# peterWon/GLoc3D

Hardware: AMD Instinct MI355X
Metric: localization queries/sec (kNN+top-20 reg), KITTI-00-sized DB (higher is better)
Workload: dtype f32

## Files before the change

### gloc3d_amd/capi.py

```python
import ctypes as C
import os

import numpy as np

HERE = os.path.dirname(os.path.abspath(__file__))
LIB_PATH = os.environ.get("GLOC3D_LIB_PATH") or os.path.join(HERE, "lib", "libgloc3d.so")

GLOC_OK = 0
ERR_NAMES = {1: "GLOC_ERR_INVALID", 2: "GLOC_ERR_HIP", 3: "GLOC_ERR_NOMEM", 4: "GLOC_ERR_NODEVICE",
             5: "GLOC_ERR_STATE"}
ALGO_AUTO, ALGO_EXACT, ALGO_MFMA, ALGO_MFMA_FP32 = 0, 1, 2, 3
KNN_OPT_ALGO, KNN_OPT_CANDIDATES, KNN_OPT_PROFILE = 1, 2, 3
REG_OPT_PROFILE, REG_OPT_NN_MODE, REG_OPT_NN_SRC_PER_LANE, REG_OPT_NN_JOB_GROUP, REG_OPT_TEMP_TARGET_INDEX = 1, 2, 3, 4, 5
REG_OPT_NN_SPLIT_HELPERS, REG_OPT_NN_SPLIT_THRESH, REG_OPT_NN_SUB_JOBS, REG_OPT_NN_HEAVY_THRESH, REG_OPT_SUB_BATCHES = 6, 7, 8, 9, 10
REG_OPT_NN_CHAIN = 11
REG_OPT_PAIRGRAPH_BUDGET = 12
REG_NN_CULLED, REG_NN_EXHAUSTIVE = 0, 1
NO_SCAN = 0xFFFFFFFF
SIZE_MAX = C.c_size_t(-1).value


class GlocError(RuntimeError):
    def __init__(self, code, msg):
        super().__init__(f"{ERR_NAMES.get(code, code)}: {msg}")
        self.code = code


class RaycastParams(C.Structure):
    _fields_ = [("n_beams", C.c_uint32), ("n_az", C.c_uint32), ("max_range", C.c_double), ("noise_sigma", C.c_double),
                ("fov_lo_deg", C.c_double), ("fov_hi_deg", C.c_double)]


class KnnStats(C.Structure):
    _fields_ = [("searches_exact", C.c_uint64), ("searches_mfma", C.c_uint64),
                ("queries_total", C.c_uint64), ("queries_fallback", C.c_uint64),
                ("last_n_tile", C.c_uint32), ("last_k_split", C.c_uint32),
                ("last_candidates", C.c_uint32)]


class RegParams(C.Structure):
    _fields_ = [("ransac_iters", C.c_uint32), ("inlier_thresh", C.c_float),
                ("min_inlier_ratio", C.c_float), ("icp_iters", C.c_uint32),
                ("max_corr_dist", C.c_float), ("seed", C.c_uint64),
                ("ransac_confidence", C.c_float), ("max_rmse", C.c_float), ("max_final_step", C.c_float)]


class NdtParams(C.Structure):
    _fields_ = [("source_leaf", C.c_float), ("resolution", C.c_float), ("step_size", C.c_float), ("trans_eps", C.c_float),
                ("max_iters", C.c_uint32), ("outlier_ratio", C.c_float), ("min_points_per_cell", C.c_uint32),
                ("min_covar_eigvalue_mult", C.c_float)]


class P2lParams(C.Structure):
    _fields_ = [("max_iters", C.c_uint32), ("max_corr_dist", C.c_float), ("trans_eps", C.c_float), ("rot_eps", C.c_float),
                ("normal_k", C.c_uint32), ("reserved_", C.c_uint32)]


class GicpParams(C.Structure):
    _fields_ = [("max_iters", C.c_uint32), ("max_corr_dist", C.c_float), ("trans_eps", C.c_float), ("rot_eps", C.c_float),
                ("normal_k", C.c_uint32), ("plane_eps", C.c_float)]


class VgicpParams(C.Structure):
    _fields_ = [("max_iters", C.c_uint32), ("max_corr_dist", C.c_float), ("trans_eps", C.c_float), ("rot_eps", C.c_float),
                ("normal_k", C.c_uint32), ("plane_eps", C.c_float), ("resolution", C.c_float), ("neighbors", C.c_uint32),
                ("min_points", C.c_uint32), ("reserved_", C.c_uint32)]


class FpfhParams(C.Structure):
# ... 993 lines not shown
    def ransac_hypotheses(self, src, tgt, corr, seed, cand, n_hyp, inlier_thresh):
        s = np.ascontiguousarray(src, np.float32).reshape(-1, 3)
        t = np.ascontiguousarray(tgt, np.float32).reshape(-1, 3)
        c = np.ascontiguousarray(corr, np.uint32)
        Rt = np.empty((n_hyp, 12), np.float32)
        valid = np.empty(n_hyp, np.uint32)
        inl = np.empty(n_hyp, np.uint32)
        check(lib().gloc_reg_ransac_hypotheses(self._h, _np_ptr(s), _np_ptr(t), _np_ptr(c),
                                               s.shape[0], seed, cand, n_hyp, _np_ptr(Rt),
                                               _np_ptr(valid), _np_ptr(inl), inlier_thresh))
        return Rt, valid, inl

    def final_steps(self, n_jobs):
        out = np.empty(n_jobs, np.float32)
        check(lib().gloc_reg_final_steps(self._h, _np_ptr(out), n_jobs))
        return out

    def nn_stats(self):
        c, n = C.c_uint64(), C.c_uint64()
        check(lib().gloc_reg_nn_stats(self._h, C.byref(c), C.byref(n)))
        return c.value, n.value

    def debug_chain(self):
        f = lib().gloc_reg_debug_chain
        f.restype = C.c_int
        f.argtypes = [C.c_void_p, C.POINTER(C.c_uint64), C.POINTER(C.c_uint64)]
        n, t = C.c_uint64(), C.c_uint64()
        check(f(self._h, C.byref(n), C.byref(t)))
        return n.value, t.value

    def debug_needed_iters(self, inl, n, conf, max_iters):
        f = lib().gloc_reg_debug_needed_iters
        f.restype = C.c_int
        f.argtypes = [C.c_void_p, C.c_void_p, C.c_void_p, C.c_uint32, C.c_float, C.c_uint32, C.c_void_p]
        a, b = np.ascontiguousarray(inl, np.uint32), np.ascontiguousarray(n, np.uint32)
        out = np.empty(a.shape[0], np.uint32)
        check(f(self._h, _np_ptr(a), _np_ptr(b), a.shape[0], conf, max_iters, _np_ptr(out)))
        return out

    def debug_chain_stall(self, on):
        f = lib().gloc_reg_debug_chain_stall
        f.restype = C.c_int
        f.argtypes = [C.c_void_p, C.c_int]
        check(f(self._h, 1 if on else 0))

    def debug_corr(self, job, n_src):
        f = lib().gloc_reg_debug_corr
        f.restype = C.c_int
        f.argtypes = [C.c_void_p, C.c_uint32, C.c_uint32, C.c_void_p, C.c_void_p]
        idx, d2 = np.empty(n_src, np.uint32), np.empty(n_src, np.float32)
        check(f(self._h, job, n_src, _np_ptr(idx), _np_ptr(d2)))
        return idx, d2


def reg_select_first_ok(ok):
    a = np.ascontiguousarray(ok, np.int32)
    return lib().gloc_reg_select_first_ok(_np_ptr(a), a.shape[0])


class NetVladFC(_Handle):

    _C = "vlad"
    set_stream, set_profile, profile = _set_stream, _set_profile, _profile

    def __init__(self, conv_w, centroids, fc_w, conv_b=None, normalize_input=True, device=0):
        cw = np.ascontiguousarray(conv_w, np.float32)
        ce = np.ascontiguousarray(centroids, np.float32)
        fw = np.ascontiguousarray(fc_w, np.float32)
        cb = None if conv_b is None else np.ascontiguousarray(conv_b, np.float32)
        self.K, self.C = cw.shape
        self.out_dim = fw.shape[1]
        assert ce.shape == (self.K, self.C) and fw.shape[0] == self.K * self.C
        self._h = C.c_void_p()
        check(lib().gloc_vlad_create(device, self.C, self.K, self.out_dim, _np_ptr(cw),
                                     None if cb is None else _np_ptr(cb), _np_ptr(ce), _np_ptr(fw),
                                     1 if normalize_input else 0, C.byref(self._h)))

    def set_gating(self, gating_w=None, scale=None, shift=None):
        if gating_w is None:
            check(lib().gloc_vlad_set_gating(self._h, None, None, None))
            return
        gw = np.ascontiguousarray(gating_w, np.float32)
        sc = np.ascontiguousarray(scale, np.float32)
        sh = np.ascontiguousarray(shift, np.float32)
        assert gw.shape == (self.out_dim, self.out_dim) and sc.shape == (self.out_dim,) == sh.shape
        check(lib().gloc_vlad_set_gating(self._h, _np_ptr(gw), _np_ptr(sc), _np_ptr(sh)))

    def forward(self, feat):
        x = np.ascontiguousarray(feat, np.float32)
        n = x.shape[0]
        x = x.reshape(n, self.C, -1)
        out = np.empty((n, self.out_dim), np.float32)
        check(lib().gloc_vlad_forward(self._h, _np_ptr(x), n, x.shape[2], _np_ptr(out)))
        return out

    def forward_device(self, feat_ptr, n, hw, out_ptr):
        check(lib().gloc_vlad_forward_device(self._h, C.c_void_p(feat_ptr), n, hw, C.c_void_p(out_ptr)))


def default_bev_params(**over):
    p = BevParams()
    check(lib().gloc_bev_default_params(C.byref(p)))
    for k, v in over.items():
        if k == "pad_bgr":
            for i in range(3):
                p.pad_bgr[i] = v[i]
# ... 458 lines not shown
```

### gloc3d_amd/csrc/reg.hip

```cpp
#include <algorithm>
#include <cmath>
#include <vector>

#include "common.hpp"

#include "fpfh.hpp"
#include "ndt.hpp"
#include "nn_compact.hpp"
#include "gicp.hpp"
#include "p2l.hpp"
#include "pairgraph.hpp"
#include "reg_kernels.hpp"
#include "scan_store.hpp"
#include "vgicp.hpp"

using namespace gloc;
using namespace gloc::reg;

struct gloc_reg : Handle {
  hipEvent_t done_ev = nullptr;
  gloc_scan_store* store = nullptr;
  gloc_scan_store* own_store = nullptr;
  DevBuf jobs, states;
  DevBuf corr, d2, pairs;
  DevBuf Rt, valid, inliers;
  DevBuf alive;
  DevBuf partials;
  DevBuf export_idx, export_d2;
  DevBuf counters;
  void* pin = nullptr;
  size_t pin_cap = 0;
  CandState* h_states = nullptr;
  Job* h_jobs = nullptr;
  struct Pending {
    bool active = false;
    std::vector<size_t> slot;
    std::vector<size_t> n_src;
    std::vector<float> def_T;
    size_t total = 0;
    float max_rmse = 0.f, max_final_step = 0.f;
    bool icp = false;
    gloc_scan_store* store = nullptr;
    std::vector<uint32_t> pinned;
  } pending;
  std::vector<float> last_final_step;
  int nn_mode = 0;
  int nn_src_per_lane = 2;
  int nn_job_group = 24;
  bool nn_job_group_set = false;
  int nn_sub_jobs = 0;
  bool temp_target_index = false;
  int nn_split_helpers = -1;
  uint32_t nn_split_thresh = 60000;
  bool nn_split_thresh_set = false;
  DevBuf split_zero, split_ff;
  NnSplit split{};
  int nn_heavy_thresh = 32;
  DevBuf heavy_buf;
  size_t heavy_cap = 0;
  NnHeavy heavy{};
  std::atomic<uint64_t> nn_launches{0};
  int nn_chain = 1;
  bool chain_broken = false;
  bool chain_stall = false;
  DevBuf chain_buf;
  uint32_t* h_chain_err = nullptr;
  bool chain_in_batch = false;
  std::vector<unsigned char> retry_jobs;
  std::vector<float> retry_T;
  gloc_reg_params retry_prm{};
  std::atomic<uint64_t> chain_launches{0}, chain_timeouts{0};
  size_t last_ld = 0;
  uint32_t last_jobs = 0;
  gloc::ndt::Ws* ndt = nullptr;
  gloc::p2l::Ws* p2l = nullptr;
  gloc::vgicp::Ws* vgicp = nullptr;
  gloc::fpfh::Ws* fpfh = nullptr;
  gloc::pairgraph::Ws* pgraph = nullptr;
  size_t pgraph_budget = 0;
  ~gloc_reg() {
    if (pending.active && pending.store) store_pin(pending.store, pending.pinned.data(), pending.pinned.size(), -1);
    if (store) store->attached--;
    if (own_store) (void)gloc_scan_store_destroy(own_store);
    gloc::ndt::ws_free(ndt);
    gloc::p2l::ws_free(p2l);
    gloc::vgicp::ws_free(vgicp);
// ... 213 lines not shown

bool batch_chains(const gloc_reg* h, const BatchDims& bd, uint32_t hx, uint32_t warm_passes) {
  if (!h->nn_chain || h->chain_broken || h->nn_mode == 1 || h->nn_src_per_lane != 2 || h->prof.enabled || NN_WPB != 1) return false;
  if (hx == 0 || warm_passes < 2) return false;
  uint32_t jg, subs;
  launch_order(h, bd.n_jobs, jg, subs);
  if (bd.n_jobs >= 48 || (jg & 7u) || jg % subs) return false;
  if ((bd.n_part & 31u) || (hx & 31u)) return false;
  const uint32_t n_wg = ((bd.max_groups + hx + NN_WPB - 1) / NN_WPB + subs - 1) / subs;
  const uint32_t groups = (bd.n_jobs * subs + jg - 1) / jg;
  const uint64_t grp_size = ((uint64_t)jg * n_wg + (jg / subs) * NN_CHAIN_ROLES + 7) & ~7ull;
  return grp_size * groups * warm_passes < (1ull << 31);
}

int launch_nn_chain(gloc_reg* h, const BatchDims& bd, const WsView& v, uint32_t n_pass, float gate2) {
  uint32_t jg, subs;
  launch_order(h, v.n_jobs, jg, subs);
  const uint32_t n_wg = ((bd.max_groups + v.split.hx + NN_WPB - 1) / NN_WPB + subs - 1) / subs;
  const uint32_t groups = (v.n_jobs * subs + jg - 1) / jg;
  NnChain ch{};
  ch.n_pass = n_pass;
  ch.expected = subs * n_wg * NN_WPB + (h->chain_stall ? 1u : 0u);
  ch.jobs_per_grp = jg / subs;
  ch.grp_size = (jg * n_wg + ch.jobs_per_grp * NN_CHAIN_ROLES + 7u) & ~7u;
  ch.pass_size = ch.grp_size * groups;
  const size_t cells = (size_t)n_pass * v.n_jobs, line = NN_CHAIN_PAD * 4;
  const size_t head = (4 * cells + 1) * line;
  const size_t t_bytes = cells * NN_CHAIN_T_STRIDE * 4;
  const size_t plan_bytes = (size_t)(n_pass - 1) * v.n_jobs * bd.n_part * 4, help_bytes = (size_t)(n_pass - 1) * v.n_jobs * v.split.hx * 4;
  const size_t sub_bytes = sizeof(double) * ACC_NV * NN_CHAIN_RED * v.n_jobs;
  GLOC_TRY(h->chain_buf.ensure(head + t_bytes + plan_bytes + help_bytes + sub_bytes + 256, v.s));
  GLOC_HIP(hipMemsetAsync(h->chain_buf.p, 0, head, v.s));
  char* base = h->chain_buf.as<char>();
  ch.ready = reinterpret_cast<uint32_t*>(base);
  ch.done = reinterpret_cast<uint32_t*>(base + cells * line);
  ch.go = reinterpret_cast<uint32_t*>(base + 2 * cells * line);
  ch.sdone = reinterpret_cast<uint32_t*>(base + 3 * cells * line);
  ch.err = reinterpret_cast<uint32_t*>(base + 4 * cells * line);
  ch.Tp = reinterpret_cast<float*>(base + head);
  ch.planp = reinterpret_cast<uint32_t*>(base + head + t_bytes);
  ch.helperp = reinterpret_cast<uint32_t*>(base + head + t_bytes + plan_bytes);
  ch.sub = reinterpret_cast<double*>(base + head + t_bytes + plan_bytes + help_bytes);
  h->nn_launches += n_pass;
  h->chain_launches++;
  h->chain_in_batch = true;
  const NnArgs a{v, bd, jg, n_wg, subs, gate2, nullptr};
  launch_compact<nn_chain_kernel<2>>(a, dim3(ch.pass_size * n_pass), v.corr, false, NnHeavy{}, ch);
  GLOC_HIP(hipGetLastError());
  GLOC_HIP(hipMemcpyAsync(h->h_chain_err, ch.err, 4, hipMemcpyDeviceToHost, v.s));
  return GLOC_OK;
}

int ensure_pinned(gloc_reg* h, uint32_t n_jobs) {
  const size_t need = (sizeof(CandState) + sizeof(Job)) * (size_t)n_jobs + 64;
  if (need > h->pin_cap) {
    if (h->pin) (void)hipHostFree(h->pin);
    h->pin = nullptr;
    h->pin_cap = 0;
    const size_t cap = need + need / 2 + 4096;
    GLOC_HIP(hipHostMalloc(&h->pin, cap, hipHostMallocDefault));
    h->pin_cap = cap;
  }
  h->h_states = reinterpret_cast<CandState*>(h->pin);
  h->h_jobs = reinterpret_cast<Job*>(h->h_states + n_jobs);
  h->h_chain_err = reinterpret_cast<uint32_t*>(h->h_jobs + n_jobs);
  return GLOC_OK;
}

struct BatchSpec {
  uint32_t n_jobs, max_src;
  uint32_t max_groups;
  bool search;
  bool pairs;
  size_t hyp;
  bool alive;
  uint32_t split_hx;
  uint32_t warm_passes;
  static BatchSpec searching(uint32_t n_jobs, size_t max_src, uint32_t max_groups) {
    return BatchSpec{n_jobs, (uint32_t)max_src, max_groups, true, false, 0, false, 0u, 0u};
  }
  static BatchSpec on_pairs(uint32_t n_jobs, size_t max_src, size_t hyp, bool alive) {
    return BatchSpec{n_jobs, (uint32_t)max_src, 0u, false, true, hyp, alive, 0u, 0u};
  }
};

struct Batch {
  BatchDims bd;
  uint32_t nblocks;
  bool chained;
  WsView v;
};

template <class Fill>
int open_batch(gloc_reg* h, const BatchSpec& sp, Batch* out, Fill&& fill) {
  const uint32_t n_jobs = sp.n_jobs;
  const int cs = h->nn_src_per_lane;
  hipStream_t s = h->stream;
  Batch& b = *out;
  b = Batch{};
  BatchDims& bd = b.bd;
  bd = BatchDims{n_jobs, sp.max_src, sp.max_groups, 0, 0};
  b.nblocks = (bd.max_src + ACC_PER_BLOCK - 1) / ACC_PER_BLOCK;
  bd.n_part = (std::max<uint32_t>(std::max(bd.max_groups, b.nblocks), 1) + 31u) & ~31u;
  bd.ld = ((size_t)bd.max_src + 127) & ~(size_t)127;
  h->last_jobs = 0;
  GLOC_TRY(ensure_pinned(h, n_jobs));
  h->chain_in_batch = false;
  *h->h_chain_err = 0u;
  fill(h->h_jobs, h->h_states);
  WsView& v = b.v;
  v.s = s;
  v.n_jobs = n_jobs;
  GLOC_TRY(h->jobs.ensure(sizeof(Job) * n_jobs, s));
  GLOC_TRY(h->states.ensure(sizeof(CandState) * n_jobs, s));
  GLOC_TRY(h->partials.ensure(sizeof(double) * ACC_NV * (size_t)bd.n_part * n_jobs, s));
  v.jobs = h->jobs.as<Job>();
  v.states = h->states.as<CandState>();
  v.partials = h->partials.as<double>();
// ... 112 lines not shown
                         (const uint32_t*)nullptr, 0u, chunk_len);
    }
    if (ph + 1 < n_ph)
      hipLaunchKernelGGL(ransac_scan_kernel<false>, dim3(n_jobs), dim3(64), 0, s, v.inliers,
                         v.valid, v.Rt, H, h0, h1, v.jobs, r.confidence,
                         r.min_inlier_ratio, v.states);
    else
      hipLaunchKernelGGL(ransac_scan_kernel<true>, dim3(n_jobs), dim3(64), 0, s, v.inliers,
                         v.valid, v.Rt, H, h0, h1, v.jobs, r.confidence,
                         r.min_inlier_ratio, v.states);
    GLOC_HIP(hipGetLastError());
  }
  return enqueue_refit(h, bd, v, thr2, nblocks);
}

int enqueue_pipeline(gloc_reg* h, const BatchDims& bd, const gloc_reg_params* prm, const WsView& v, bool can, bool any_tgt,
                     uint32_t nblocks, bool chained) {
  const uint32_t n_jobs = v.n_jobs;
  hipStream_t s = v.s;
  const bool culled = h->nn_mode != 1;
  const float gate2 = prm->max_corr_dist > 0.f ? prm->max_corr_dist * prm->max_corr_dist : 0.f;
  bool have_corr = false;

  if (can && any_tgt && prm->ransac_iters > 0) {
    GLOC_TRY(launch_nn(h, bd, v, false, true, 0.f));
    have_corr = true;
    GLOC_TRY(enqueue_ransac(h, bd, RansacRule{prm->ransac_iters, prm->inlier_thresh, prm->min_inlier_ratio, prm->ransac_confidence, prm->seed},
                            v, nblocks));
  }
  for (uint32_t it = 0; it < prm->icp_iters && can && any_tgt; ++it) {
    if (chained && have_corr) {
      GLOC_TRY(launch_nn_chain(h, bd, v, prm->icp_iters - it, gate2));
      break;
    }
    GLOC_TRY(launch_nn(h, bd, v, have_corr, false, gate2));
    have_corr = true;
    if (!culled) {
      ProfScope ps(h->prof, "accum", s);
      hipLaunchKernelGGL(accum_kernel<0>, dim3(nblocks, n_jobs), dim3(ACC_THREADS), 0, s, v.jobs,
                         v.states, v.corr, v.d2,
                         (const f32x4*)nullptr, bd.ld, gate2, v.partials, bd.n_part);
      GLOC_HIP(hipGetLastError());
    }
    {
      ProfScope ps(h->prof, "solve", s);
      hipLaunchKernelGGL(solve_kernel<0>, dim3(v.split.hx ? 2 * n_jobs : n_jobs), dim3(SOLVE_THREADS), 0, s, v.partials,
                         bd.n_part, culled, v.jobs, v.states, v.split, n_jobs);
      GLOC_HIP(hipGetLastError());
    }
  }
  return GLOC_OK;
}

int enqueue_jobs(gloc_reg* h, const std::vector<JobHost>& jh, const gloc_reg_params* prm) {
  const uint32_t n_jobs = (uint32_t)jh.size();
  if (n_jobs == 0) return GLOC_OK;
  const int cs = h->nn_src_per_lane;
  uint32_t max_src = 0;
  bool can = false, any_tgt = false;
  for (const JobHost& j : jh) {
    max_src = std::max<uint32_t>(max_src, (uint32_t)j.src.n);
    can |= j.src.n >= 3;
    any_tgt |= j.tgt.n >= 1;
  }
  const bool ransac = can && any_tgt && prm->ransac_iters > 0;
  const bool adaptive = prm->ransac_confidence > 0.f && prm->ransac_confidence < 1.f;
  const uint32_t warm_passes = !(can && any_tgt) ? 0u : (ransac ? prm->icp_iters : std::max<uint32_t>(prm->icp_iters, 1u) - 1u);
  BatchSpec spec = BatchSpec::searching(n_jobs, max_src, src_groups(max_src, cs));
  spec.pairs = ransac;
  spec.hyp = prm->ransac_iters;
  spec.alive = !adaptive;
  spec.split_hx = split_helpers(h, n_jobs);
  spec.warm_passes = warm_passes;
  Batch b;
  GLOC_TRY(open_batch(h, spec, &b, [&](Job* jd, CandState* st) {
    for (uint32_t c = 0; c < n_jobs; ++c) {
      const DevScan &s = jh[c].src, &t = jh[c].tgt;
      jd[c] = Job{s.idx.pts, s.order, s.idx.inv, t.xyz, t.idx, (uint32_t)s.n, src_groups(s.n, cs), jh[c].stream_id, 0u};
      init_state(st[c], jh[c].init_T, prm->ransac_iters);
      if (s.n < 3) st[c].frozen = 1;
    }
  }));
  hipStream_t s = h->stream;
  GLOC_TRY(enqueue_pipeline(h, b.bd, prm, b.v, can, any_tgt, b.nblocks, b.chained));
  GLOC_HIP(hipMemcpyAsync(h->h_states, h->states.p, sizeof(CandState) * n_jobs, hipMemcpyDeviceToHost, s));
  GLOC_HIP(hipEventRecord(h->done_ev, s));
  if (h->chain_in_batch) {
    h->retry_jobs.resize(sizeof(JobHost) * n_jobs);
    memcpy(h->retry_jobs.data(), jh.data(), sizeof(JobHost) * n_jobs);
    h->retry_T.assign((size_t)16 * n_jobs, 0.f);
    for (uint32_t c = 0; c < n_jobs; ++c)
      if (jh[c].init_T) memcpy(&h->retry_T[(size_t)16 * c], jh[c].init_T, sizeof(float) * 16);
    h->retry_prm = *prm;
  }
  return GLOC_OK;
}

int collect_jobs(gloc_reg* h, uint32_t n_jobs, const size_t* n_src_of, float max_rmse, float max_final_step, float* out_T,
                 float* out_rmse, uint32_t* out_inliers, int* out_ok) {
  h->last_final_step.assign(n_jobs, 0.f);
  if (n_jobs == 0) return GLOC_OK;
  GLOC_HIP(hipEventSynchronize(h->done_ev));
  if (h->chain_in_batch && *h->h_chain_err) {
    const bool first = !h->chain_broken;
    h->chain_broken = true;
    h->chain_timeouts++;
    if (first)
      fprintf(stderr, "[gloc3d] the chained ICP passes of a batch of %u jobs timed out on the device (a wait for a job's solve ran out): "
                      "the batch is run again launch by launch, and this handle launches pass by pass from now on\n", n_jobs);
    GLOC_REQUIRE(h->retry_jobs.size() == sizeof(JobHost) * n_jobs, GLOC_ERR_HIP,
                 "the chained ICP passes of a batch of %u jobs timed out on the device and the batch cannot be run again", n_jobs);
    std::vector<JobHost> jh(n_jobs);
    memcpy(jh.data(), h->retry_jobs.data(), sizeof(JobHost) * n_jobs);
    for (uint32_t c = 0; c < n_jobs; ++c)
      if (jh[c].init_T) jh[c].init_T = &h->retry_T[(size_t)16 * c];
    const gloc_reg_params prm = h->retry_prm;
    if (const int rc = enqueue_jobs(h, jh, &prm)) {
      (void)hipStreamSynchronize(h->stream);
      return rc;
    }
    GLOC_HIP(hipEventSynchronize(h->done_ev));
  }
  for (uint32_t c = 0; c < n_jobs; ++c) {
    const CandState& st = h->h_states[c];
    const size_t n_src = n_src_of[c];
    pose_to_T16(st, out_T + 16 * (size_t)c);
    const float rmse = n_src ? (float)std::sqrt(st.sum_d2 / (double)n_src) : 0.f;
    if (out_rmse) out_rmse[c] = rmse;
    if (out_inliers) out_inliers[c] = st.best_inl;
    h->last_final_step[c] = st.last_step;
    if (out_ok)
      out_ok[c] = st.ok && !(max_rmse > 0.f && !(rmse <= max_rmse)) && !(max_final_step > 0.f && !(st.last_step <= max_final_step));
  }
  return GLOC_OK;
}

int run_jobs(gloc_reg* h, const std::vector<JobHost>& jh, const gloc_reg_params* prm, float* out_T, float* out_rmse,
             uint32_t* out_inliers, int* out_ok) {
  GLOC_TRY(enqueue_jobs(h, jh, prm));
  std::vector<size_t> n_src(jh.size());
  for (size_t c = 0; c < jh.size(); ++c) n_src[c] = jh[c].src.n;
  return collect_jobs(h, (uint32_t)jh.size(), n_src.data(), prm->max_rmse, prm->icp_iters ? prm->max_final_step : 0.f, out_T,
                      out_rmse, out_inliers, out_ok);
}

// ... 418 lines not shown
  }
  if (option == GLOC_REG_OPT_NN_MODE) {
    GLOC_REQUIRE(value == GLOC_REG_NN_CULLED || value == GLOC_REG_NN_EXHAUSTIVE, GLOC_ERR_INVALID,
                 "bad nn mode %lld", (long long)value);
    h->nn_mode = (int)value;
    return GLOC_OK;
  }
  if (option == GLOC_REG_OPT_NN_JOB_GROUP) {
    GLOC_REQUIRE(value >= 1 && value <= 65536, GLOC_ERR_INVALID, "must be in [1, 65536]");
    h->nn_job_group = (int)value;
    h->nn_job_group_set = true;
    return GLOC_OK;
  }
  if (option == GLOC_REG_OPT_TEMP_TARGET_INDEX) {
    h->temp_target_index = value != 0;
    return GLOC_OK;
  }
  if (option == GLOC_REG_OPT_NN_SUB_JOBS) {
    GLOC_REQUIRE(value >= 0 && value <= 64, GLOC_ERR_INVALID, "must be in [0, 64]");
    h->nn_sub_jobs = (int)value;
    return GLOC_OK;
  }
  if (option == GLOC_REG_OPT_NN_SPLIT_HELPERS) {
    GLOC_REQUIRE(value >= -1 && value <= 4096, GLOC_ERR_INVALID, "must be in [-1, 4096]");
    h->nn_split_helpers = (int)value;
    return GLOC_OK;
  }
  if (option == GLOC_REG_OPT_SUB_BATCHES) {
    GLOC_REQUIRE(value >= -1 && value <= 8, GLOC_ERR_INVALID, "must be in [-1, 8]");
    return GLOC_OK;
  }
  if (option == GLOC_REG_OPT_NN_CHAIN) {
    GLOC_REQUIRE(value == 0 || value == 1, GLOC_ERR_INVALID, "must be 0 or 1");
    h->nn_chain = (int)value;
    if (value) h->chain_broken = false;
    return GLOC_OK;
  }
  if (option == GLOC_REG_OPT_NN_HEAVY_THRESH) {
    GLOC_REQUIRE(value >= 0 && value <= 65535, GLOC_ERR_INVALID, "must be in [0, 65535]");
    h->nn_heavy_thresh = (int)value;
    return GLOC_OK;
  }
  if (option == GLOC_REG_OPT_NN_SPLIT_THRESH) {
    GLOC_REQUIRE(value >= 0 && value <= 0x3FFFFFFF, GLOC_ERR_INVALID, "must be in [0, 2^30)");
    h->nn_split_thresh = (uint32_t)value;
    h->nn_split_thresh_set = true;
    return GLOC_OK;
  }
  if (option == GLOC_REG_OPT_NN_SRC_PER_LANE) {
    GLOC_REQUIRE(value == 1 || value == 2 || value == 4, GLOC_ERR_INVALID, "must be 1, 2 or 4");
    h->nn_src_per_lane = (int)value;
    return GLOC_OK;
  }
  if (option == GLOC_REG_OPT_PAIRGRAPH_BUDGET) {
    GLOC_REQUIRE(value >= 0 && (uint64_t)value <= gloc::pairgraph::BUDGET_BYTES, GLOC_ERR_INVALID, "must be in [0, 2^30]");
    h->pgraph_budget = (size_t)value;
    return GLOC_OK;
  }
  set_err("unknown option %d", option);
  return GLOC_ERR_INVALID;
}

int gloc_reg_scan_upload(gloc_reg* h, const float* pts, size_t n, size_t stride_floats,
                         uint32_t* scan_id) {
  GLOC_REQUIRE(h, GLOC_ERR_INVALID, "null handle");
  GLOC_HIP(hipSetDevice(h->device));
  GLOC_TRY(ensure_store(h));
  return gloc_scan_store_add(h->store, pts, n, stride_floats, scan_id);
}

int gloc_reg_scan_build_target_index(gloc_reg* h, uint32_t scan_id) {
  GLOC_REQUIRE(h, GLOC_ERR_INVALID, "null handle");
  GLOC_REQUIRE(h->store, GLOC_ERR_INVALID, "unknown scan id %u", scan_id);
  GLOC_HIP(hipSetDevice(h->device));
  GLOC_HIP(hipStreamSynchronize(h->stream));
  return gloc_scan_store_build_target_index(h->store, scan_id);
}

int gloc_reg_scan_release(gloc_reg* h, uint32_t scan_id) {
  GLOC_REQUIRE(h, GLOC_ERR_INVALID, "null handle");
  GLOC_REQUIRE(h->store, GLOC_ERR_INVALID, "unknown scan id %u", scan_id);
  GLOC_HIP(hipSetDevice(h->device));
  GLOC_HIP(hipStreamSynchronize(h->stream));
  return gloc_scan_store_release(h->store, scan_id);
}

int gloc_reg_scan_count(const gloc_reg* h, size_t* n_scans) {
  GLOC_REQUIRE(h && n_scans, GLOC_ERR_INVALID, "null argument");
  *n_scans = 0;
  if (!h->store) return GLOC_OK;
  return gloc_scan_store_count(h->store, n_scans);
}

int gloc_reg_batch(gloc_reg* h, const float* q_xyz, size_t nq_pts, const float* const* cand_xyz,
                   const size_t* cand_npts, size_t n_cand, const uint32_t* cand_stream_ids,
                   const float* init_T, const gloc_reg_params* params, float* out_T,
                   float* out_rmse, uint32_t* out_inliers, int* out_ok) {
  GLOC_REQUIRE(h && out_T && (q_xyz || nq_pts == 0), GLOC_ERR_INVALID, "null argument");
  GLOC_REQUIRE(n_cand >= 1 && n_cand <= 4096 && cand_xyz && cand_npts, GLOC_ERR_INVALID,
               "n_cand = %zu outside [1,4096] or null candidate arrays", n_cand);
  GLOC_REQUIRE(nq_pts < (1ull << 31), GLOC_ERR_INVALID, "query scan too large");
  GLOC_NOT_PENDING(h);
  GLOC_TRY(check_params(params));
  GLOC_HIP(hipSetDevice(h->device));
  for (size_t c = 0; c < n_cand; ++c) {
    GLOC_REQUIRE(cand_xyz[c] || cand_npts[c] == 0, GLOC_ERR_INVALID, "candidate %zu is null", c);
// ... 280 lines not shown
  GLOC_HIP(hipMemcpyAsync(v.pairs, hp.data(), sizeof(float) * hp.size(), hipMemcpyHostToDevice, s));
  GLOC_HIP(hipMemsetAsync(v.inliers, 0, sizeof(uint32_t) * (size_t)n_hyp, s));
  hipLaunchKernelGGL(ransac_hyp_kernel, dim3((n_hyp + 127) / 128, 1), dim3(128), 0, s, v.pairs, ld, v.jobs, seed, n_hyp, 0u, n_hyp,
                     (const CandState*)nullptr, v.Rt, v.valid);
  GLOC_HIP(hipGetLastError());
  dim3 grid((n_hyp + 255) / 256, (unsigned)((n + SC_CHUNK - 1) / SC_CHUNK), 1);
  hipLaunchKernelGGL(ransac_score_kernel, grid, dim3(256), 0, s, v.pairs, ld, v.jobs, n_hyp, 0u, 256u , v.Rt,
                     v.valid, inlier_thresh * inlier_thresh, (const CandState*)nullptr, v.inliers, (const uint32_t*)nullptr,
                     (const uint32_t*)nullptr, 0u, (uint32_t)SC_CHUNK);
  GLOC_HIP(hipGetLastError());
  GLOC_HIP(hipMemcpyAsync(out_Rt, v.Rt, sizeof(float) * 12 * (size_t)n_hyp, hipMemcpyDeviceToHost, s));
  GLOC_HIP(hipMemcpyAsync(out_valid, v.valid, sizeof(uint32_t) * (size_t)n_hyp, hipMemcpyDeviceToHost, s));
  GLOC_HIP(hipMemcpyAsync(out_inliers, v.inliers, sizeof(uint32_t) * (size_t)n_hyp, hipMemcpyDeviceToHost, s));
  GLOC_HIP(hipStreamSynchronize(s));
  return GLOC_OK;
}

int gloc_reg_nn_stats(gloc_reg* h, uint64_t* pairs_evaluated, uint64_t* launches) {
  GLOC_REQUIRE(h, GLOC_ERR_INVALID, "null handle");
  GLOC_HIP(hipSetDevice(h->device));
  unsigned long long c = 0;
  if (h->counters.p) {
    std::vector<unsigned long long> part(NN_STAT_SLOTS);
    GLOC_HIP(hipMemcpyAsync(part.data(), h->counters.p, 8 * NN_STAT_SLOTS, hipMemcpyDeviceToHost, h->stream));
    GLOC_HIP(hipStreamSynchronize(h->stream));
    for (unsigned long long v : part) c += v;
  }
  if (pairs_evaluated) *pairs_evaluated = c;
  if (launches) *launches = h->nn_launches;
  return GLOC_OK;
}

int gloc_reg_debug_corr(gloc_reg* h, uint32_t job, uint32_t n_src, uint32_t* out_idx, float* out_d2) {
  GLOC_REQUIRE(h && out_idx && out_d2, GLOC_ERR_INVALID, "null argument");
  GLOC_HIP(hipSetDevice(h->device));
  hipStream_t s = h->stream;
  const size_t ld = h->last_ld;
  GLOC_NOT_PENDING(h);
  GLOC_REQUIRE(job < h->last_jobs && n_src <= ld, GLOC_ERR_INVALID, "no such job in the last batch");
  GLOC_TRY(h->export_idx.ensure(sizeof(uint32_t) * ld * h->last_jobs, s));
  GLOC_TRY(h->export_d2.ensure(sizeof(float) * ld * h->last_jobs, s));
  hipLaunchKernelGGL(export_corr_kernel, dim3((unsigned)((ld + 255) / 256), h->last_jobs), dim3(256), 0, s,
                     h->jobs.as<Job>(), h->corr.as<uint32_t>(), h->d2.as<float>(), ld,
                     h->export_idx.as<uint32_t>(), h->export_d2.as<float>());
  GLOC_HIP(hipGetLastError());
  GLOC_HIP(hipMemcpyAsync(out_idx, h->export_idx.as<uint32_t>() + (size_t)job * ld, sizeof(uint32_t) * n_src,
                          hipMemcpyDeviceToHost, s));
  GLOC_HIP(hipMemcpyAsync(out_d2, h->export_d2.as<float>() + (size_t)job * ld, sizeof(float) * n_src,
                          hipMemcpyDeviceToHost, s));
  GLOC_HIP(hipStreamSynchronize(s));
  return GLOC_OK;
}

int gloc_reg_debug_chain(gloc_reg* h, uint64_t* launches, uint64_t* timeouts) {
  GLOC_REQUIRE(h, GLOC_ERR_INVALID, "null handle");
  if (launches) *launches = h->chain_launches;
  if (timeouts) *timeouts = h->chain_timeouts;
  return GLOC_OK;
}

int gloc_reg_debug_needed_iters(gloc_reg* h, const uint32_t* inl, const uint32_t* n, uint32_t count, float conf, uint32_t max_iters,
                                uint32_t* out) {
  GLOC_REQUIRE(h && inl && n && out, GLOC_ERR_INVALID, "null argument");
  GLOC_HIP(hipSetDevice(h->device));
  GLOC_NOT_PENDING(h);
  hipStream_t s = h->stream;
  GLOC_TRY(h->export_idx.ensure(sizeof(uint32_t) * 3 * (size_t)count, s));
  uint32_t* d = h->export_idx.as<uint32_t>();
  GLOC_HIP(hipMemcpyAsync(d, inl, 4 * (size_t)count, hipMemcpyHostToDevice, s));
  GLOC_HIP(hipMemcpyAsync(d + count, n, 4 * (size_t)count, hipMemcpyHostToDevice, s));
  hipLaunchKernelGGL(needed_iters_kernel, dim3((count + 255) / 256), dim3(256), 0, s, d, d + count, conf, max_iters, d + 2 * (size_t)count, count);
  GLOC_HIP(hipGetLastError());
  GLOC_HIP(hipMemcpyAsync(out, d + 2 * (size_t)count, 4 * (size_t)count, hipMemcpyDeviceToHost, s));
  GLOC_HIP(hipStreamSynchronize(s));
  return GLOC_OK;
}

int gloc_reg_debug_chain_stall(gloc_reg* h, int on) {
  GLOC_REQUIRE(h, GLOC_ERR_INVALID, "null handle");
  h->chain_stall = on != 0;
  return GLOC_OK;
}

int gloc_reg_ndt_batch_ids(gloc_reg* h, uint32_t src_scan_id, const uint32_t* tgt_scan_ids, size_t n, const float* init_T,
                           const gloc_ndt_params* prm, float* out_T, double* out_prob, uint32_t* out_iters,
                           int* out_converged) {
  GLOC_REQUIRE(h && out_T && tgt_scan_ids, GLOC_ERR_INVALID, "null argument");
  GLOC_NOT_PENDING(h);
  GLOC_HIP(hipSetDevice(h->device));
  return gloc::ndt::run(ndt_ctx(h), src_scan_id, tgt_scan_ids, n, init_T, nullptr, prm, out_T, out_prob, out_iters, out_converged,
                        nullptr);
}

int gloc_reg_ndt_derivatives(gloc_reg* h, uint32_t src_scan_id, uint32_t tgt_scan_id, const double p6[6],
                             const gloc_ndt_params* prm, double* out_score, double* out_grad6, double* out_hess36) {
  GLOC_REQUIRE(h && p6 && out_score && out_grad6 && out_hess36, GLOC_ERR_INVALID, "null argument");
  GLOC_NOT_PENDING(h);
  GLOC_HIP(hipSetDevice(h->device));
  double s[43];
  GLOC_TRY(gloc::ndt::run(ndt_ctx(h), src_scan_id, &tgt_scan_id, 1, nullptr, p6, prm, nullptr, nullptr, nullptr, nullptr, s));
  *out_score = s[0];
  for (int i = 0; i < 6; ++i) out_grad6[i] = s[1 + i];
  for (int i = 0; i < 36; ++i) out_hess36[i] = s[7 + i];
  return GLOC_OK;
}

// ... 161 lines not shown
```

### include/gloc3d.h

```cpp
#ifndef GLOC3D_H
#define GLOC3D_H

#include <stddef.h>
#include <stdint.h>

#ifdef __cplusplus
extern "C" {
#endif

#define GLOC3D_ABI_VERSION 6

enum {
  GLOC_OK = 0,
  GLOC_ERR_INVALID = 1,
  GLOC_ERR_HIP = 2,
  GLOC_ERR_NOMEM = 3,
  GLOC_ERR_NODEVICE = 4,
  GLOC_ERR_STATE = 5
};

const char* gloc_last_error(void);
int gloc_abi_version(void);
int gloc_device_count(void);

// ... 51 lines not shown
int gloc_knn_search_sharded(gloc_knn* h, gloc_comm* comm, const float* d_queries, size_t nq, size_t k,
                            uint64_t index_stride, uint64_t index_offset, uint64_t* d_out_idx,
                            float* d_out_d2);

int gloc_knn_search_sharded_host(gloc_knn* h, gloc_comm* comm, const float* queries, size_t nq, size_t k,
                                 uint64_t index_stride, uint64_t index_offset, uint64_t* out_idx,
                                 float* out_d2);
int gloc_comm_all_gather_host(gloc_comm* c, const void* send, void* recv, size_t bytes_per_rank);

typedef struct gloc_knn_stats {
  uint64_t searches_exact, searches_mfma, queries_total, queries_fallback;
  uint32_t last_n_tile, last_k_split, last_candidates;
} gloc_knn_stats;
int gloc_knn_get_stats(const gloc_knn* h, gloc_knn_stats* out);

int gloc_knn_profile(gloc_knn* h, const char* kernel, double* total_ms, uint64_t* launches);
int gloc_knn_profile_reset(gloc_knn* h);

typedef struct gloc_reg gloc_reg;

typedef struct gloc_reg_params {
  uint32_t ransac_iters;
  float inlier_thresh;
  float min_inlier_ratio;
  uint32_t icp_iters;
  float max_corr_dist;
  uint64_t seed;
  float ransac_confidence;
  float max_rmse;
  float max_final_step;
} gloc_reg_params;

#define GLOC_REG_FINAL_STEP_SUGGESTED 0.03f

void gloc_reg_default_params(gloc_reg_params* p);

int gloc_reg_create(int device, gloc_reg** out);
int gloc_reg_destroy(gloc_reg* h);
int gloc_reg_set_stream(gloc_reg* h, void* hip_stream);
int gloc_reg_synchronize(gloc_reg* h);
int gloc_reg_set_option(gloc_reg* h, int option, int64_t value);
enum {
  GLOC_REG_OPT_PROFILE = 1,
  GLOC_REG_OPT_NN_MODE = 2,
  GLOC_REG_OPT_NN_SRC_PER_LANE = 3,
  GLOC_REG_OPT_NN_JOB_GROUP = 4,
  GLOC_REG_OPT_TEMP_TARGET_INDEX = 5,
  GLOC_REG_OPT_NN_SPLIT_HELPERS = 6,
  GLOC_REG_OPT_NN_SPLIT_THRESH = 7,
  GLOC_REG_OPT_NN_SUB_JOBS = 8,
  GLOC_REG_OPT_NN_HEAVY_THRESH = 9,
  GLOC_REG_OPT_SUB_BATCHES = 10,
  GLOC_REG_OPT_NN_CHAIN = 11,
  GLOC_REG_OPT_PAIRGRAPH_BUDGET = 12
};
enum {
  GLOC_REG_NN_CULLED = 0,
  GLOC_REG_NN_EXHAUSTIVE = 1
};

typedef struct gloc_scan_store gloc_scan_store;
int gloc_scan_store_create(int device, gloc_scan_store** out);
int gloc_scan_store_destroy(gloc_scan_store* st);
int gloc_scan_store_add(gloc_scan_store* st, const float* pts, size_t n, size_t stride_floats,
                        uint32_t* scan_id);
int gloc_scan_store_add_device(gloc_scan_store* st, const float* d_pts, size_t n,
                               size_t stride_floats, uint32_t* scan_id);
int gloc_scan_store_add_batch(gloc_scan_store* st, const float* const* pts, const size_t* n, size_t count,
                              size_t stride_floats, uint32_t* scan_ids);
int gloc_scan_store_build_target_index(gloc_scan_store* st, uint32_t scan_id);
int gloc_scan_store_build_target_index_batch(gloc_scan_store* st, const uint32_t* scan_ids, size_t count);
int gloc_scan_store_release(gloc_scan_store* st, uint32_t scan_id);
int gloc_scan_store_clear(gloc_scan_store* st);
int gloc_scan_store_count(gloc_scan_store* st, size_t* n_scans);
int gloc_scan_store_bytes(gloc_scan_store* st, size_t* live_bytes, size_t* cached_bytes);
int gloc_scan_store_points(gloc_scan_store* st, uint32_t scan_id, size_t* n_points);
int gloc_scan_store_download(gloc_scan_store* st, uint32_t scan_id, float* out_xyz,
                             size_t capacity_points);
int gloc_scan_store_build_normals(gloc_scan_store* st, uint32_t scan_id, uint32_t k );
int gloc_scan_store_normals(gloc_scan_store* st, uint32_t scan_id, float* out_nxyz, size_t capacity_points);

int gloc_reg_attach_store(gloc_reg* h, gloc_scan_store* store);

int gloc_reg_scan_upload(gloc_reg* h, const float* pts, size_t n, size_t stride_floats,
                         uint32_t* scan_id);
int gloc_reg_scan_build_target_index(gloc_reg* h, uint32_t scan_id);
int gloc_reg_scan_release(gloc_reg* h, uint32_t scan_id);
int gloc_reg_scan_count(const gloc_reg* h, size_t* n_scans);
int gloc_reg_scan_clear(gloc_reg* h);

int gloc_reg_batch(gloc_reg* h, const float* q_xyz, size_t nq_pts, const float* const* cand_xyz,
                   const size_t* cand_npts, size_t n_cand, const uint32_t* cand_stream_ids,
                   const float* init_T, const gloc_reg_params* params, float* out_T,
                   float* out_rmse, uint32_t* out_inliers, int* out_ok);

int gloc_reg_batch_ids(gloc_reg* h, uint32_t q_scan_id, const uint32_t* cand_scan_ids,
                       size_t n_cand, const uint32_t* cand_stream_ids, const float* init_T,
                       const gloc_reg_params* params, float* out_T, float* out_rmse,
                       uint32_t* out_inliers, int* out_ok);

int gloc_reg_batch_multi(gloc_reg* h, size_t n_queries, const uint32_t* q_scan_ids,
                         const uint32_t* cand_scan_ids, size_t n_cand,
                         const uint32_t* cand_stream_ids, const float* init_T,
                         const gloc_reg_params* params, float* out_T, float* out_rmse,
                         uint32_t* out_inliers, int* out_ok);

int gloc_reg_batch_multi_begin(gloc_reg* h, size_t n_queries, const uint32_t* q_scan_ids,
// ... 396 lines not shown
```

Measured before the change: 593.7.

## Regroup source points spatially per batch and sort groups by extent for NN

Result: faster. 601.5 (median of 6 runs) (+1.3%).

```diff
diff --git a/gloc3d_amd/capi.py b/gloc3d_amd/capi.py
--- a/gloc3d_amd/capi.py
+++ b/gloc3d_amd/capi.py
@@ -15,6 +15,7 @@
 REG_OPT_NN_SPLIT_HELPERS, REG_OPT_NN_SPLIT_THRESH, REG_OPT_NN_SUB_JOBS, REG_OPT_NN_HEAVY_THRESH, REG_OPT_SUB_BATCHES = 6, 7, 8, 9, 10
 REG_OPT_NN_CHAIN = 11
 REG_OPT_PAIRGRAPH_BUDGET = 12
+REG_OPT_SRC_GROUPING = 13
 REG_NN_CULLED, REG_NN_EXHAUSTIVE = 0, 1
 NO_SCAN = 0xFFFFFFFF
 SIZE_MAX = C.c_size_t(-1).value
@@ -1114,6 +1115,20 @@
         check(f(self._h, job, n_src, _np_ptr(idx), _np_ptr(d2)))
         return idx, d2
 
+    def debug_src_view(self, scan_id, n, src_per_lane=2, batch=None):
+        f = lib().gloc_reg_debug_src_view
+        f.restype = C.c_int
+        f.argtypes = [C.c_void_p, C.c_void_p, C.c_size_t, C.c_size_t, C.c_void_p, C.c_void_p, C.POINTER(C.c_int)]
+        ids = np.ascontiguousarray([scan_id] if batch is None else batch, np.uint32)
+        which = int(np.nonzero(ids == scan_id)[0][0])
+        ng = (n + 64 * src_per_lane - 1) // (64 * src_per_lane)
+        perm, order = np.empty(max(n, 1), np.uint32), np.empty(max(ng, 1), np.uint32)
+        has = C.c_int()
+        check(f(self._h, _np_ptr(ids), ids.shape[0], which, _np_ptr(perm), _np_ptr(order), C.byref(has)))
+        if not has.value:
+            return None
+        return dict(perm=perm[:n], order=order[:ng])
+
 
 def reg_select_first_ok(ok):
     a = np.ascontiguousarray(ok, np.int32)
diff --git a/gloc3d_amd/csrc/reg.hip b/gloc3d_amd/csrc/reg.hip
--- a/gloc3d_amd/csrc/reg.hip
+++ b/gloc3d_amd/csrc/reg.hip
@@ -1,5 +1,6 @@
 #include <algorithm>
 #include <cmath>
+#include <map>
 #include <vector>
 
 #include "common.hpp"
@@ -12,6 +13,8 @@
 #include "pairgraph.hpp"
 #include "reg_kernels.hpp"
 #include "scan_store.hpp"
+#include "seg_sort.hpp"
+#include "src_view.hpp"
 #include "vgicp.hpp"
 
 using namespace gloc;
@@ -32,6 +35,9 @@
   size_t pin_cap = 0;
   CandState* h_states = nullptr;
   Job* h_jobs = nullptr;
+  SrcView* h_views = nullptr;
+  int src_grouping = 1;
+  DevBuf view_pts, view_idx, view_desc;
   struct Pending {
     bool active = false;
     std::vector<size_t> slot;
@@ -351,7 +357,7 @@
 }
 
 int ensure_pinned(gloc_reg* h, uint32_t n_jobs) {
-  const size_t need = (sizeof(CandState) + sizeof(Job)) * (size_t)n_jobs + 64;
+  const size_t need = (sizeof(CandState) + sizeof(Job) + sizeof(SrcView) + sizeof(segsort::Seg)) * (size_t)n_jobs + 64;
   if (need > h->pin_cap) {
     if (h->pin) (void)hipHostFree(h->pin);
     h->pin = nullptr;
@@ -363,6 +369,7 @@
   h->h_states = reinterpret_cast<CandState*>(h->pin);
   h->h_jobs = reinterpret_cast<Job*>(h->h_states + n_jobs);
   h->h_chain_err = reinterpret_cast<uint32_t*>(h->h_jobs + n_jobs);
+  h->h_views = reinterpret_cast<SrcView*>(reinterpret_cast<char*>(h->h_jobs + n_jobs) + 64);
   return GLOC_OK;
 }
 
@@ -581,10 +588,78 @@
   return GLOC_OK;
 }
 
-int enqueue_jobs(gloc_reg* h, const std::vector<JobHost>& jh, const gloc_reg_params* prm) {
+int build_src_views(gloc_reg* h, std::vector<JobHost>& jh, int cs) {
+  if (!h->src_grouping || h->nn_mode == 1) return GLOC_OK;
+  hipStream_t s = h->stream;
   const uint32_t n_jobs = (uint32_t)jh.size();
+  GLOC_TRY(ensure_pinned(h, n_jobs));
+  std::vector<segsort::Seg> segs;
+  std::vector<uint32_t> view_of(n_jobs, 0xFFFFFFFFu);
+  std::map<const void*, uint32_t> seen;
+  std::vector<size_t> pts_off;
+  size_t n_pts = 0;
+  uint32_t n_views = 0, max_blocks = 0, n_grp = 0;
+  for (uint32_t c = 0; c < n_jobs; ++c) {
+    const DevScan& sc = jh[c].src;
+    const uint32_t ng = src_groups(sc.n, cs);
+    if (sc.kd || sc.n == 0 || !sc.order || ng > SV_MAX_GROUPS) continue;
+    auto it = seen.find(sc.idx.pts);
+    if (it == seen.end()) {
+      it = seen.emplace(sc.idx.pts, n_views).first;
+      h->h_views[n_views] = SrcView{sc.idx.pts, nullptr, nullptr, nullptr, nullptr, nullptr, (uint32_t)sc.n, ng, 64u * (uint32_t)cs, 0u};
+      segs.push_back(segsort::Seg{n_grp, ng});
+      pts_off.push_back(n_pts);
+      n_pts += sc.n;
+      n_grp += ng;
+      max_blocks = std::max<uint32_t>(max_blocks, (uint32_t)((sc.n + SV_BLOCK - 1) / SV_BLOCK));
+      ++n_views;
+    }
+    view_of[c] = it->second;
+  }
+  if (!n_views) return GLOC_OK;
+  GLOC_TRY(h->view_pts.ensure(sizeof(f32x4) * n_pts, s));
+  GLOC_TRY(h->view_idx.ensure(sizeof(uint32_t) * (n_pts + 3 * (size_t)n_grp), s));
+  GLOC_TRY(h->view_desc.ensure((sizeof(SrcView) + sizeof(segsort::Seg)) * n_views, s));
+  uint32_t* d_order = h->view_idx.as<uint32_t>() + n_pts;
+  uint32_t* d_key = d_order + n_grp;
+  uint32_t* d_id = d_key + n_grp;
+  for (uint32_t v = 0; v < n_views; ++v) {
+    SrcView& sv = h->h_views[v];
+    sv.out_pts = h->view_pts.as<f32x4>() + pts_off[v];
+    sv.out_inv = h->view_idx.as<uint32_t>() + pts_off[v];
+    sv.out_order = d_order + segs[v].begin;
+    sv.out_key = d_key + segs[v].begin;
+    sv.out_id = d_id + segs[v].begin;
+  }
+  memcpy(h->h_views + n_views, segs.data(), sizeof(segsort::Seg) * n_views);
+  GLOC_HIP(hipMemcpyAsync(h->view_desc.p, h->h_views, (sizeof(SrcView) + sizeof(segsort::Seg)) * n_views, hipMemcpyHostToDevice, s));
+  const SrcView* d_views = h->view_desc.as<SrcView>();
+  const segsort::Seg* d_segs = reinterpret_cast<const segsort::Seg*>(d_views + n_views);
+  {
+    ProfScope ps(h->prof, "src_view", s);
+    for (uint32_t v0 = 0; v0 < n_views; v0 += 65535u) {
+      const uint32_t nv = std::min<uint32_t>(n_views - v0, 65535u);
+      hipLaunchKernelGGL(src_view_regroup_kernel, dim3(max_blocks, nv), dim3(SV_THREADS), 0, s, d_views + v0);
+    }
+    hipLaunchKernelGGL(segsort::small_sort_kernel, dim3(n_views), dim3(1024), 0, s, d_key, d_id, d_segs, d_order);
+    GLOC_HIP(hipGetLastError());
+  }
+  for (uint32_t c = 0; c < n_jobs; ++c) {
+    if (view_of[c] == 0xFFFFFFFFu) continue;
+    const SrcView& sv = h->h_views[view_of[c]];
+    jh[c].src.idx.pts = sv.out_pts;
+    jh[c].src.idx.inv = sv.out_inv;
+    jh[c].src.order = sv.out_order;
+  }
+  return GLOC_OK;
+}
+
+int enqueue_jobs(gloc_reg* h, const std::vector<JobHost>& jh_store, const gloc_reg_params* prm) {
+  const uint32_t n_jobs = (uint32_t)jh_store.size();
   if (n_jobs == 0) return GLOC_OK;
   const int cs = h->nn_src_per_lane;
+  std::vector<JobHost> jh = jh_store;
+  GLOC_TRY(build_src_views(h, jh, cs));
   uint32_t max_src = 0;
   bool can = false, any_tgt = false;
   for (const JobHost& j : jh) {
@@ -616,10 +691,10 @@
   GLOC_HIP(hipEventRecord(h->done_ev, s));
   if (h->chain_in_batch) {
     h->retry_jobs.resize(sizeof(JobHost) * n_jobs);
-    memcpy(h->retry_jobs.data(), jh.data(), sizeof(JobHost) * n_jobs);
+    memcpy(h->retry_jobs.data(), jh_store.data(), sizeof(JobHost) * n_jobs);
     h->retry_T.assign((size_t)16 * n_jobs, 0.f);
     for (uint32_t c = 0; c < n_jobs; ++c)
-      if (jh[c].init_T) memcpy(&h->retry_T[(size_t)16 * c], jh[c].init_T, sizeof(float) * 16);
+      if (jh_store[c].init_T) memcpy(&h->retry_T[(size_t)16 * c], jh_store[c].init_T, sizeof(float) * 16);
     h->retry_prm = *prm;
   }
   return GLOC_OK;
@@ -1144,6 +1219,11 @@
     h->nn_src_per_lane = (int)value;
     return GLOC_OK;
   }
+  if (option == GLOC_REG_OPT_SRC_GROUPING) {
+    GLOC_REQUIRE(value == 0 || value == 1, GLOC_ERR_INVALID, "must be 0 or 1");
+    h->src_grouping = (int)value;
+    return GLOC_OK;
+  }
   if (option == GLOC_REG_OPT_PAIRGRAPH_BUDGET) {
     GLOC_REQUIRE(value >= 0 && (uint64_t)value <= gloc::pairgraph::BUDGET_BYTES, GLOC_ERR_INVALID, "must be in [0, 2^30]");
     h->pgraph_budget = (size_t)value;
@@ -1530,6 +1610,38 @@
   return GLOC_OK;
 }
 
+int gloc_reg_debug_src_view(gloc_reg* h, const uint32_t* scan_ids, size_t n_ids, size_t which, uint32_t* out_perm, uint32_t* out_order,
+                            int* has_view) {
+  GLOC_REQUIRE(h && scan_ids && out_perm && out_order && has_view, GLOC_ERR_INVALID, "null argument");
+  GLOC_REQUIRE(n_ids >= 1 && n_ids <= 65536 && which < n_ids, GLOC_ERR_INVALID, "n_ids = %zu outside [1, 65536] or which = %zu past it", n_ids, which);
+  GLOC_REQUIRE(h->store, GLOC_ERR_INVALID, "no scan store");
+  GLOC_NOT_PENDING(h);
+  GLOC_HIP(hipSetDevice(h->device));
+  hipStream_t s = h->stream;
+  const int cs = h->nn_src_per_lane;
+  const std::vector<int> css(n_ids, cs);
+  ScopedPins pins(h->store, s);
+  GLOC_TRY(pins.pin(scan_ids, css.data(), n_ids));
+  std::vector<JobHost> jh(n_ids);
+  for (size_t c = 0; c < n_ids; ++c) jh[c] = JobHost{pins.scans[c], DevScan{}, 0u, nullptr};
+  h->last_jobs = 0;
+  const int keep = h->src_grouping;
+  h->src_grouping = 1;
+  const int rc = build_src_views(h, jh, cs);
+  h->src_grouping = keep;
+  GLOC_TRY(rc);
+  const DevScan& sv = jh[which].src;
+  *has_view = sv.idx.pts != pins.scans[which].idx.pts;
+  if (!*has_view) return GLOC_OK;
+  const size_t n = sv.n;
+  std::vector<f32x4> pts(n);
+  GLOC_HIP(hipMemcpyAsync(pts.data(), sv.idx.pts, sizeof(f32x4) * n, hipMemcpyDeviceToHost, s));
+  GLOC_HIP(hipMemcpyAsync(out_order, sv.order, sizeof(uint32_t) * src_groups(n, cs), hipMemcpyDeviceToHost, s));
+  GLOC_HIP(hipStreamSynchronize(s));
+  for (size_t i = 0; i < n; ++i) memcpy(&out_perm[i], reinterpret_cast<const char*>(&pts[i]) + 12, 4);
+  return GLOC_OK;
+}
+
 int gloc_reg_debug_chain(gloc_reg* h, uint64_t* launches, uint64_t* timeouts) {
   GLOC_REQUIRE(h, GLOC_ERR_INVALID, "null handle");
   if (launches) *launches = h->chain_launches;
diff --git a/gloc3d_amd/csrc/src_view.hpp b/gloc3d_amd/csrc/src_view.hpp
--- /dev/null
+++ b/gloc3d_amd/csrc/src_view.hpp
@@ -0,0 +1,180 @@
+#pragma once
+#include <hip/hip_runtime.h>
+#include <stdint.h>
+
+#include "scan_index.hpp"
+
+namespace gloc {
+namespace reg {
+
+#ifndef GLOC_SV_BLOCK
+#define GLOC_SV_BLOCK 4096
+#endif
+constexpr uint32_t SV_BLOCK = GLOC_SV_BLOCK;
+constexpr uint32_t SV_LEAF = 128;
+constexpr uint32_t SV_THREADS = SV_BLOCK / 4;
+constexpr uint32_t SV_MAX_GROUPS = 4096;
+constexpr int SV_LEVELS = SV_BLOCK == 4096 ? 5 : 4;
+static_assert(SV_BLOCK == 2048 || SV_BLOCK == 4096, "block sizes with four positions per lane and at most 1024 threads");
+static_assert((SV_BLOCK >> SV_LEVELS) == SV_LEAF && SV_BLOCK <= 65536, "levels down to the leaf; 16-bit offsets");
+
+struct SrcView {
+  const f32x4* pts;
+  f32x4* out_pts;
+  uint32_t* out_inv;
+  uint32_t* out_order;
+  uint32_t* out_key;
+  uint32_t* out_id;
+  uint32_t n, n_groups, group, pad_;
+};
+
+__global__ __launch_bounds__(SV_THREADS) void src_view_regroup_kernel(const SrcView* __restrict__ views) {
+  constexpr int E = SV_BLOCK / SV_THREADS;
+  constexpr uint32_t MAX_NODES = 1u << (SV_LEVELS - 1), WSPAN = 64 * E;
+  static_assert(SV_LEAF * 2 >= WSPAN && E % 2 == 0, "a wave's positions lie in one node at every level");
+  __shared__ unsigned long long a[SV_BLOCK];
+  __shared__ uint32_t blo[MAX_NODES][3], bhi[MAX_NODES][3], nskip[MAX_NODES];
+  const SrcView v = views[blockIdx.y];
+  const uint32_t base = blockIdx.x * SV_BLOCK;
+  if (base >= v.n) return;
+  const uint32_t tid = threadIdx.x, lane = tid & 63u, wbase = (tid >> 6) * WSPAN;
+  const f32x4* __restrict__ pts = v.pts;
+  uint32_t src[E];
+  int prev_axis = -1;
+#pragma unroll
+  for (int e = 0; e < E; ++e) src[e] = wbase + 64 * e + lane;
+  for (int level = 0; level < SV_LEVELS; ++level) {
+    const uint32_t node_shift = 31 - __builtin_clz(SV_BLOCK) - level, node_size = 1u << node_shift;
+    const uint32_t node = wbase >> node_shift;
+    if (tid < MAX_NODES * 3) {
+      blo[tid / 3][tid % 3] = 0xFFFFFFFFu;
+      bhi[tid / 3][tid % 3] = 0u;
+    }
+    __syncthreads();
+    float c[E][3];
+    bool real[E];
+    {
+      float lo[3] = {3.4e38f, 3.4e38f, 3.4e38f}, hi[3] = {-3.4e38f, -3.4e38f, -3.4e38f};
+      bool any_l = false;
+#pragma unroll
+      for (int e = 0; e < E; ++e) {
+        real[e] = base + src[e] < v.n;
+        c[e][0] = c[e][1] = c[e][2] = 0.f;
+        if (real[e]) {
+          const f32x4 p = pts[base + src[e]];
+          c[e][0] = p.x; c[e][1] = p.y; c[e][2] = p.z;
+#pragma unroll
+          for (int k = 0; k < 3; ++k) {
+            lo[k] = fminf(lo[k], c[e][k]);
+            hi[k] = fmaxf(hi[k], c[e][k]);
+          }
+          any_l = true;
+        }
+      }
+      const bool any = __builtin_amdgcn_ballot_w64(any_l) != 0ull;
+      for (int o = 32; o > 0; o >>= 1)
+#pragma unroll
+        for (int k = 0; k < 3; ++k) {
+          lo[k] = fminf(lo[k], __shfl_xor(lo[k], o));
+          hi[k] = fmaxf(hi[k], __shfl_xor(hi[k], o));
+        }
+      if (lane == 0 && any) {
+#pragma unroll
+        for (int k = 0; k < 3; ++k) {
+          atomicMin(&blo[node][k], f2ord(lo[k]));
+          atomicMax(&bhi[node][k], f2ord(hi[k]));
+        }
+      }
+    }
+    __syncthreads();
+    const float ex = ord2f(bhi[node][0]) - ord2f(blo[node][0]), ey = ord2f(bhi[node][1]) - ord2f(blo[node][1]),
+                ez = ord2f(bhi[node][2]) - ord2f(blo[node][2]);
+    int axis = 0;
+    float ext = ex;
+    if (ey > ext) { axis = 1; ext = ey; }
+    if (ez > ext) axis = 2;
+    const bool wskip = axis == prev_axis;
+    prev_axis = axis;
+    if (lane == 0) nskip[node] = wskip ? 1u : 0u;
+#pragma unroll
+    for (int e = 0; e < E; ++e) {
+      const uint32_t i = wbase + 64 * e + lane;
+      const uint32_t key = real[e] ? f2ord(axis == 0 ? c[e][0] : (axis == 1 ? c[e][1] : c[e][2])) : 0xFFFFFFFFu;
+      a[i] = ((unsigned long long)key << 32) | ((unsigned long long)i << 16) | src[e];
+    }
+    for (uint32_t k = 2; k <= node_size; k <<= 1) {
+      for (uint32_t j = k >> 1; j > 0; j >>= 1) {
+        const bool mirror = j == (k >> 1), cross = j >= WSPAN;
+        if (cross) __syncthreads();
+        else {
+          __builtin_amdgcn_fence(__ATOMIC_RELEASE, "wavefront");
+          __builtin_amdgcn_wave_barrier();
+          __builtin_amdgcn_fence(__ATOMIC_ACQUIRE, "wavefront");
+        }
+#pragma unroll
+        for (int e = 0; e < E / 2; ++e) {
+          const uint32_t q = (wbase >> 1) + 64 * e + lane;
+          const uint32_t i = ((q & ~(j - 1u)) << 1) | (q & (j - 1u));
+          const uint32_t p = mirror ? (i ^ (k - 1u)) : (i | j);
+          if (cross ? nskip[i >> node_shift] != 0u : wskip) continue;
+          const unsigned long long x = a[i], y = a[p];
+          if (x > y) {
+            a[i] = y;
+            a[p] = x;
+          }
+        }
+        if (cross) __syncthreads();
+      }
+    }
+    __builtin_amdgcn_fence(__ATOMIC_RELEASE, "wavefront");
+    __builtin_amdgcn_wave_barrier();
+    __builtin_amdgcn_fence(__ATOMIC_ACQUIRE, "wavefront");
+#pragma unroll
+    for (int e = 0; e < E; ++e) src[e] = (uint32_t)a[wbase + 64 * e + lane] & 0xFFFFu;
+    __syncthreads();
+  }
+  float glo[E][3], ghi[E][3];
+#pragma unroll
+  for (int e = 0; e < E; ++e) {
+    const uint32_t slot = base + wbase + 64 * e + lane;
+#pragma unroll
+    for (int k = 0; k < 3; ++k) glo[e][k] = 3.4e38f, ghi[e][k] = -3.4e38f;
+    if (slot < v.n) {
+      const f32x4 p = pts[base + src[e]];
+      v.out_pts[slot] = p;
+      v.out_inv[__float_as_uint(p.w)] = slot;
+      glo[e][0] = ghi[e][0] = p.x; glo[e][1] = ghi[e][1] = p.y; glo[e][2] = ghi[e][2] = p.z;
+    }
+    for (int o = 32; o > 0; o >>= 1)
+#pragma unroll
+      for (int k = 0; k < 3; ++k) {
+        glo[e][k] = fminf(glo[e][k], __shfl_xor(glo[e][k], o));
+        ghi[e][k] = fmaxf(ghi[e][k], __shfl_xor(ghi[e][k], o));
+      }
+  }
+  if (lane == 0) {
+    const uint32_t cpg = v.group / 64u;
+    static_assert(E == 4, "the folds below are written out for four chunks per wave");
+    auto fold = [&](int to, int from) {
+#pragma unroll
+      for (int k = 0; k < 3; ++k) {
+        glo[to][k] = fminf(glo[to][k], glo[from][k]);
+        ghi[to][k] = fmaxf(ghi[to][k], ghi[from][k]);
+      }
+    };
+    if (cpg >= 2u) { fold(0, 1); fold(2, 3); }
+    if (cpg == 4u) fold(0, 2);
+#pragma unroll
+    for (int e = 0; e < E; ++e) {
+      const uint32_t first = base + wbase + 64 * e;
+      if ((uint32_t)e % cpg == 0u && first < v.n) {
+        const float dx = ghi[e][0] - glo[e][0], dy = ghi[e][1] - glo[e][1], dz = ghi[e][2] - glo[e][2];
+        v.out_key[first / v.group] = ~f2ord(dx * dx + dy * dy + dz * dz);
+        v.out_id[first / v.group] = first / v.group;
+      }
+    }
+  }
+}
+
+}
+}
diff --git a/include/gloc3d.h b/include/gloc3d.h
--- a/include/gloc3d.h
+++ b/include/gloc3d.h
@@ -127,7 +127,8 @@
   GLOC_REG_OPT_NN_HEAVY_THRESH = 9,
   GLOC_REG_OPT_SUB_BATCHES = 10,
   GLOC_REG_OPT_NN_CHAIN = 11,
-  GLOC_REG_OPT_PAIRGRAPH_BUDGET = 12
+  GLOC_REG_OPT_PAIRGRAPH_BUDGET = 12,
+  GLOC_REG_OPT_SRC_GROUPING = 13
 };
 enum {
   GLOC_REG_NN_CULLED = 0,
```
